# DaviGuanabara/dronechase

Measured on AMD Instinct MI355X. Metric: env-steps/sec (whole job), random-action rollout, higher is better.
Workload: dtype f32

## Files before the change

dronechase_amd/csrc/te_env.hip:

```cpp
#include <hip/hip_runtime.h>
#include <hip/hip_ext.h>

#include <algorithm>
#include <cmath>
#include <cstdio>
#include <cstdlib>
#include <cstring>
#include <map>
#include <mutex>
#include <new>
#include <string>
#include <tuple>
#include <type_traits>
#include <vector>

#include "te_logic.hpp"
#include "te_stacked.hpp"
#include "te_stackview.hpp"
#include "te_engage.hpp"
#include "te_engage_slots.hpp"
#include "te_policy.hpp"
#include "te_policy_bf16.hpp"
#include "te_sphere.hpp"
#include "te_wingman.hpp"
#include "te_policy_grad.hpp"
#include "te_policy_grad_bf16.hpp"
#include "te_policy_opt.hpp"
#include "te_rollout.hpp"
#include "te_monitor.hpp"

namespace te {

#ifndef TE_K1_BLOCK
#define TE_K1_BLOCK 64
#endif
constexpr long long kHelpMaxPairs = 98304;
#ifdef TE_K1_WAVES
#define TE_K1_ATTR __attribute__((amdgpu_waves_per_eu(TE_K1_WAVES, TE_K1_WAVES)))
#else
#define TE_K1_ATTR
#endif
typedef uint32_t te_u4 __attribute__((ext_vector_type(4)));
struct FillJob { float* lidar; uint32_t total_quads; uint32_t n_fill_waves; uint32_t mode; const uint16_t* prev; uint32_t lists, list_rows, npad, n, tile_words; };

struct NavView {
  const SlotLane& P; int Pn;
  TE_DEV float gf(int w, int s) const { return P.lf_slot(TE_X_REF + (w - TE_D_OBS_POS), s); }
};

constexpr int kEagerP = 4;
struct RegNav {
  float ref[3][kEagerP];
  TE_DEV float gf(int w, int s) const {
    float v = 0.0f;
#pragma unroll
    for (int q = 0; q < kEagerP; ++q) v = s == q ? ref[w - TE_D_OBS_POS][q] : v;
    return v;
  }
};
template <int FAMILY, bool NOISE, bool MIXED, bool CES = true, bool HELP = false, bool EAGER = false>
TE_DEV void fly(const Params& p, const float* __restrict__ actions, int slot, int env, bool valid, const float* nzbuf = nullptr, const volatile int* ready = nullptr, uint32_t gate = 1u) {
  const int D = p.D;
  const SlotLane P(p.dstate, p.estate, (uint32_t)D, (uint32_t)p.Npad, (uint32_t)slot, (uint32_t)env,
                   (uint32_t)(TE_DRONE_WORDS + TE_X_WORDS) * (uint32_t)D * (uint32_t)p.Npad, (uint32_t)TE_ENV_WORDS * (uint32_t)p.Npad);
  int armed = EAGER ? 0 : P.li(TE_D_ARMED);
  const bool want = EAGER ? valid : (valid && armed != 0);
  const te_config& c = p.cfg;
  const bool mode7 = (FAMILY == FAM_STAGE01) && slot == 2;
  uint32_t nav_S = 0u; int nav_state = 0; V3 nav_me{0, 0, 0}; RegNav rnav;
#pragma unroll
  for (int k = 0; k < 3; ++k)
#pragma unroll
    for (int q = 0; q < kEagerP; ++q) rnav.ref[k][q] = 0.0f;

  float4 act = make_float4(0, 0, 0, 0);
  float cmd[4] = {0, 0, 0, 0};
// ... 134 lines not shown
#undef TE_DRAW

  const M3 R = x_rotation(b.q);
  if (!c.observe_lag) {
    b.o_pos = b.pos; b.o_vel = mulT(R, b.vel); b.o_rate = b.wb; b.o_eul = euler_of(b.q);
  }
  const V3 ww = mul(R, b.wb);
  P.sf(TE_D_POS, b.pos.x); P.sf(TE_D_POS + 1, b.pos.y); P.sf(TE_D_POS + 2, b.pos.z);
  P.sf(TE_D_QUAT, b.q.x); P.sf(TE_D_QUAT + 1, b.q.y); P.sf(TE_D_QUAT + 2, b.q.z); P.sf(TE_D_QUAT + 3, b.q.w);
  P.sf(TE_D_VEL, b.vel.x); P.sf(TE_D_VEL + 1, b.vel.y); P.sf(TE_D_VEL + 2, b.vel.z);
  P.sf(TE_D_OMEGA, ww.x); P.sf(TE_D_OMEGA + 1, ww.y); P.sf(TE_D_OMEGA + 2, ww.z);
#pragma unroll
  for (int k = 0; k < 4; ++k) P.sf(TE_D_THROTTLE + k, b.thr[k]);
#pragma unroll
  for (int k = 0; k < 3; ++k) { P.sf(TE_D_PID_AV_I + k, b.av_i[k]); P.sf(TE_D_PID_AV_E + k, b.av_e[k]); }
#pragma unroll
  for (int k = 0; k < 2; ++k) { P.sf(TE_D_PID_LV_I + k, b.lv_i[k]); P.sf(TE_D_PID_LV_E + k, b.lv_e[k]); }
  P.sf(TE_D_PID_ZV_I, b.zv_i); P.sf(TE_D_PID_ZV_E, b.zv_e);
  P.sf(TE_D_OBS_POS, b.o_pos.x); P.sf(TE_D_OBS_POS + 1, b.o_pos.y); P.sf(TE_D_OBS_POS + 2, b.o_pos.z);
  P.sf(TE_D_OBS_EULER, b.o_eul.x); P.sf(TE_D_OBS_EULER + 1, b.o_eul.y); P.sf(TE_D_OBS_EULER + 2, b.o_eul.z);
  P.sf(TE_D_OBS_VEL, b.o_vel.x); P.sf(TE_D_OBS_VEL + 1, b.o_vel.y); P.sf(TE_D_OBS_VEL + 2, b.o_vel.z);
  P.sf(TE_D_OBS_RATE, b.o_rate.x); P.sf(TE_D_OBS_RATE + 1, b.o_rate.y); P.sf(TE_D_OBS_RATE + 2, b.o_rate.z);
  if (mode7) {
#pragma unroll
    for (int k = 0; k < 6; ++k) P.sf(TE_D_PENDING + k, 0.0f);
  }
}

#ifdef TE_DEBUG_STAMPS
#define TE_K1_BASE(p) (64 + 16 * (size_t)((p).Npad / kEPB + 1))
#define TE_K1_BEGIN const unsigned long long k1_t0_ = __builtin_amdgcn_s_memrealtime();
#define TE_K1_END(kind)                                                                                               \
  do {                                                                                                                \
    if (p.dbg && threadIdx.x == 0) {                                                                                  \
      asm volatile("s_waitcnt vmcnt(0) lgkmcnt(0)" ::: "memory");                                                    \
      unsigned long long* r_ = p.dbg + TE_K1_BASE(p) + 4 * (size_t)blockIdx.x;                                        \
      r_[0] = k1_t0_; r_[1] = __builtin_amdgcn_s_memrealtime();                                                       \
      r_[2] = (unsigned long long)__builtin_amdgcn_s_getreg((31 << 11) | 4) | ((unsigned long long)__builtin_amdgcn_s_getreg((31 << 11) | 20) << 32); \
      r_[3] = (kind);                                                                                                 \
    }                                                                                                                 \
  } while (0)
#else
#define TE_K1_BEGIN
#define TE_K1_END(kind) do {} while (0)
#endif

template <int FAMILY, bool EAGER>
TE_DEV void noise_help(const Params& p, int slot, int env, bool valid, float* nzbuf, volatile int* ready, uint32_t gate) {
  const te_config& c = p.cfg;
  const int lane = threadIdx.x & 63;
  const SlotLane P(p.dstate, p.estate, (uint32_t)p.D, (uint32_t)p.Npad, (uint32_t)slot, (uint32_t)env,
                   (uint32_t)(TE_DRONE_WORDS + TE_X_WORDS) * (uint32_t)p.D * (uint32_t)p.Npad, (uint32_t)TE_ENV_WORDS * (uint32_t)p.Npad);
  const int armed = P.li(TE_D_ARMED);
  const uint32_t episode = (uint32_t)P.lei(TE_E_EPISODE);
  const uint32_t step_index = (uint32_t)P.lei(TE_E_STEP) + (FAMILY == FAM_STAGE01 ? 1u : 0u);
  if (EAGER) {
    if (!gate) return;
    if (lane == 0) *ready = 0;
    asm volatile("s_waitcnt lgkmcnt(0)\n\ts_barrier" ::: "memory");
  }
  if (__ballot(valid && armed != 0) == 0ull) return;
  const int S = c.substeps;
  for (int s = 0; s < S; s += 2) {
    const U4 bits = motor_noise_bits(c, env, slot, episode, step_index, s);
    float nz[4];
    motor_noise_from(bits.x, bits.y, p.kd.noise_m2ln2, nz);
    *reinterpret_cast<float4*>(nzbuf + ((size_t)s * 64 + lane) * 4) = make_float4(nz[0], nz[1], nz[2], nz[3]);
    if (s + 1 < S) {
      motor_noise_from(bits.z, bits.w, p.kd.noise_m2ln2, nz);
      *reinterpret_cast<float4*>(nzbuf + ((size_t)(s + 1) * 64 + lane) * 4) = make_float4(nz[0], nz[1], nz[2], nz[3]);
    }
    asm volatile("s_waitcnt lgkmcnt(0)" ::: "memory");
    if (lane == 0) *ready = min(s + 2, S);
  }
}

template <int FAMILY, bool NOISE, bool FILL, bool CES = true, bool HELP = false>
__global__ __launch_bounds__(HELP ? 128 : TE_K1_BLOCK) TE_K1_ATTR void substeps_kernel(Params p, const float* __restrict__ actions, FillJob fill) {
  TE_K1_BEGIN
  extern __shared__ float k1_lds[];
  int wave = HELP ? (int)blockIdx.x : __builtin_amdgcn_readfirstlane((int)((blockIdx.x * (unsigned)TE_K1_BLOCK + threadIdx.x) >> 6));
  const int role = HELP ? __builtin_amdgcn_readfirstlane((int)(threadIdx.x >> 6)) : 0;
  volatile int* ready = reinterpret_cast<volatile int*>(k1_lds + (HELP ? (size_t)p.cfg.substeps * 256 : 0));
  const int lane = threadIdx.x & 63;
  const int D = p.D;
  const int nchunks = p.Npad >> 6;
  float4* fill_dst = reinterpret_cast<float4*>(fill.lidar);
  if (FILL) {
    if (HELP && role == 1 && wave < (int)fill.n_fill_waves) return;
    if (wave < (int)fill.n_fill_waves && fill.mode == 3) {
      const uint32_t nch = fill.npad >> 6;
      const uint32_t list = (uint32_t)wave / nch, env = ((uint32_t)wave - list * nch) * 64u + (uint32_t)lane;
      if (env < fill.n) {
        const uint16_t* __restrict__ pv = fill.prev + (size_t)list * fill.list_rows * fill.npad + env;
        float* d0 = fill.lidar + ((size_t)env * fill.lists + list) * fill.tile_words;
        const int cnt = (int)pv[0];
        const bool time_plane = fill.tile_words > 2u * TE_LIDAR_CELLS;
        for (int pl = 0; pl < (time_plane ? 3 : 2); ++pl)
          for (int i = 0; i < cnt; ++i) d0[pl * TE_LIDAR_CELLS + pv[(size_t)(1 + i) * fill.npad]] = 1.0f;
      }
      TE_K1_END(1);
      return;
    }
    if (wave < (int)fill.n_fill_waves) {
      if (fill.mode >= 1) {
        const uint32_t n_blocks = fill.total_quads >> 6;
        const __amdgpu_buffer_rsrc_t rs = __builtin_amdgcn_make_buffer_rsrc(fill.lidar, 0, (int)(n_blocks << 10), 0x00020000);
        const int voff = lane * 16;
        const te_u4 ones = {0x3f800000u, 0x3f800000u, 0x3f800000u, 0x3f800000u};
        for (uint32_t b = (uint32_t)wave; b < n_blocks; b += fill.n_fill_waves)
          __builtin_amdgcn_raw_buffer_store_b128(ones, rs, voff, (int)(b << 10), 2 );
        const uint32_t q = (n_blocks << 6) + (uint32_t)lane;
        if ((uint32_t)wave == n_blocks % fill.n_fill_waves && q < fill.total_quads) TE_FILL_STORE(fill_dst + q);
        TE_K1_END(1);
        return;
      }
      const uint32_t stride = fill.n_fill_waves * 64u;
      for (uint32_t q = (uint32_t)wave * 64u + (uint32_t)lane; q < fill.total_quads; q += stride) TE_FILL_STORE(fill_dst + q);
      TE_K1_END(1);
      return;
    }
    wave -= (int)fill.n_fill_waves;
  }
  const int n_head = min(D, p.cfg.n_pursuers + 1) * nchunks;
  const int n_mixed = (FAMILY == FAM_LEVEL4 && p.dense_min > 1) ? kMixedWaves * nchunks : 0;
  if (wave >= n_head && wave < n_head + n_mixed) {
    wave -= n_head;
    const int m = wave / nchunks, chunk = wave - m * nchunks;
    const int count = __builtin_amdgcn_readfirstlane((int)((const uint32_t* __restrict__)p.mixed_count)[chunk]);
    if (m * 64 >= count) { TE_K1_END(0); return; }
    const int i = m * 64 + lane;
    const bool valid = i < count;
    const uint32_t item = valid ? (uint32_t)p.mixed_items[(size_t)chunk * kMixedCap + i] : 0u;
    if (HELP && role == 1) { noise_help<FAMILY, true>(p, (int)(item >> 8), chunk * 64 + (int)(item & 63u), valid, k1_lds, ready, 1u); return; }
    fly<FAMILY, NOISE, true, CES, HELP, HELP>(p, actions, (int)(item >> 8), chunk * 64 + (int)(item & 63u), valid, k1_lds, ready);
    TE_K1_END(3);
    return;
  }
  if (wave >= n_head) wave -= n_mixed;
  const int slot = wave / nchunks;
  const int chunk = wave - slot * nchunks;
  if (slot >= D) { TE_K1_END(0); return; }
  const uint32_t* __restrict__ sm32 = reinterpret_cast<const uint32_t*>(p.slot_mask);
  const uint32_t chunk_mask = __builtin_amdgcn_readfirstlane(sm32[2 * chunk + (slot >> 5)]);
  const int env = chunk * 64 + lane;
  if (HELP && FAMILY == FAM_LEVEL4) {
    const uint32_t gate = (chunk_mask >> (slot & 31)) & 1u;
// ... 269 lines not shown
}
__global__ void init_planes(Params p) {
  for (size_t i = blockIdx.x * (size_t)blockDim.x + threadIdx.x; i < (size_t)p.D * p.Npad; i += (size_t)gridDim.x * blockDim.x)
    reinterpret_cast<float*>(p.dstate)[(size_t)(TE_D_QUAT + 3) * p.D * p.Npad + i] = 1.0f;
}
__global__ void random_actions_kernel(Params p, float* __restrict__ actions, uint64_t seed, uint64_t step_index) {
  int env = blockIdx.x * blockDim.x + threadIdx.x;
  if (env >= p.N) return;
  uint64_t g = (uint64_t)p.cfg.env_index_base + (uint64_t)env;
  U4 r = philox4x32_10((uint32_t)g, RNG_ACTION | ((uint32_t)(g >> 32) << 24), (uint32_t)step_index, (uint32_t)(step_index >> 32),
                       (uint32_t)seed, (uint32_t)(seed >> 32));
  reinterpret_cast<float4*>(actions)[env] = make_float4(-1.0f + 2.0f * u01(r.x), -1.0f + 2.0f * u01(r.y), -1.0f + 2.0f * u01(r.z), u01(r.w));
}

}

using namespace te;

template <typename... Args> struct Launch { void (*fn)(Args...) = nullptr; const char* name = ""; unsigned block = 0; size_t lds = 0; };
#define TE_KERNEL(...) &__VA_ARGS__, #__VA_ARGS__

struct KernelPlan {
  Launch<Params, const float*, FillJob> substeps[2];
  Launch<Params, const float*, StepOut> engage;
  Launch<StackParams> ring_push;
  Launch<StackParams, StackOut> stack_view;
  size_t observe_lds = 0;
  Launch<Params, int, float*, float*, float*, uint8_t*> wingman_one;
  Launch<Params, int, float*, uint32_t, uint32_t, float*, float*, uint8_t*, uint32_t*> wingman_view;
  Launch<Params, float*, const uint32_t*> wingman_patch;
  uint32_t wingman_fill_waves = 256;
  bool records_cells = false;
  int n_fill_waves = 256, dense_min = kDenseMin;
};
static int family_of(int task) {
  return task == TE_TASK_STAGE01 ? FAM_STAGE01 : (task == TE_TASK_STAGE02 ? FAM_STAGE02 : FAM_LEVEL4);
}
template <typename F>
static void launch_by_family(int family, F&& f) {
  switch (family) {
    case FAM_STAGE01: f(std::integral_constant<int, FAM_STAGE01>{}); break;
    case FAM_STAGE02: f(std::integral_constant<int, FAM_STAGE02>{}); break;
    default: f(std::integral_constant<int, FAM_LEVEL4>{}); break;
  }
}
template <typename F> static void with_bool(bool b, F&& f) { if (b) f(std::true_type{}); else f(std::false_type{}); }
template <int FAMILY, bool NOISE, bool FILL, bool CES, bool HELP>
static Launch<Params, const float*, FillJob> substep_role(const te_config& c) {
  static const std::string name = "substeps_kernel<" + std::to_string(FAMILY) + (NOISE ? ", true" : ", false") + (FILL ? ", true" : ", false") +
                                  (CES ? ", true" : ", false") + (HELP ? ", true>" : ", false>");
  return {&substeps_kernel<FAMILY, NOISE, FILL, CES, HELP>, name.c_str(), HELP ? 128u : (unsigned)TE_K1_BLOCK, HELP ? (size_t)c.substeps * 1024 + 16 : 0};
}

static const char* check_config(const te_config* cfg) {
  if (cfg->struct_size != sizeof(te_config)) return "te_create: te_config.struct_size mismatch (ABI skew)";
  const int D = cfg->n_pursuers + cfg->n_invaders;
  if (cfg->n_envs < 1) return "te_create: n_envs < 1";
  if (cfg->n_pursuers < 1 || cfg->n_invaders < 1 || D > kMaxD64 || cfg->n_pursuers > 31) return "te_create: need 1 <= P <= 31, 1 <= I, P + I <= 64";
  if (cfg->initial_invaders < 0 || cfg->invaders_per_round < 0) return "te_create: initial_invaders / invaders_per_round must not be negative";
  if (cfg->substeps < 0 || cfg->substeps > 255) return "te_create: substeps out of range";
  if (cfg->substeps == 0 && cfg->observe_lag != 0) return "te_create: substeps == 0 (no physics) needs observe_lag == 0";
  if (cfg->task < TE_TASK_STAGE01 || cfg->task > TE_TASK_LEVEL5_FUSION) return "te_create: unknown task";
  if (cfg->ground_contact && family_of(cfg->task) != FAM_LEVEL4) return "te_create: cfg.ground_contact is built for the level4 task family only";
  if (cfg->evaluation && (((uint32_t)cfg->evaluation >> 8) >> cfg->n_pursuers) != 0u) return "te_create: cfg.evaluation's driver mask names a pursuer that does not exist";
  if (cfg->evaluation && !(family_of(cfg->task) == FAM_LEVEL4 && cfg->ally_policy == TE_ALLY_BT && !cfg->stacked_obs))
    return "te_create: cfg.evaluation (Evaluation_Task rules) is the level4 task family with behaviour-tree drivers and the own-sphere observation";
// ... 51 lines not shown
  else if (spw && !c.stacked_obs) k.engage = {TE_KERNEL(engage_slots_multi_kernel<2, true, false>), multi_block, multi_lds};
  else if (spw == 1) k.engage = {TE_KERNEL(engage_slots_multi_kernel<1, false, false>), multi_block, multi_lds};
  else if (spw == 2) k.engage = {TE_KERNEL(engage_slots_multi_kernel<2, false, false>), multi_block, multi_lds};
  else if (spw == 3) k.engage = {TE_KERNEL(engage_slots_multi_kernel<3, false, false>), multi_block, multi_lds};
  else if (regs_s2 && !eng_regs) k.engage = {TE_KERNEL(engage_slots_stage02_kernel<16>), 64u * D, slot_lds};
  else if (slots) k.engage = {TE_KERNEL(engage_slots_kernel<16>), 64u * D, slot_lds};
#ifndef TE_DEBUG_STAMPS
  else if (contact && P <= 2 && D <= 11) k.engage = {TE_KERNEL(engage_kernel<2, 9, true>), 64, 0};
  else if (contact) k.engage = {TE_KERNEL(engage_kernel<6, 12, true>), 64, 0};
#endif
  else if (regs_l4 && P <= 2 && D <= 11) k.engage = {TE_KERNEL(engage_kernel<2, 9, false>), 64, 0};
  else if (regs_l4 && P <= 6 && D <= 18) k.engage = {TE_KERNEL(engage_kernel<6, 12, false>), 64, 0};
  else if (regs_l4) k.engage = {TE_KERNEL(engage_kernel<7, 30, false>), 64, 0};
  else if (regs_s2) k.engage = {TE_KERNEL(engage_stage02_kernel<2, 8>), 64, 0};
  else if (regs_s1) k.engage = {TE_KERNEL(engage_stage01_kernel), 64, 0};
  else if (l4 && lds > 53 * 1024) k.engage = {TE_KERNEL(engage_observe_kernel<0, 512>), 512, lds};
  else if (l4) k.engage = {TE_KERNEL(engage_observe_kernel<0, 256>), 256, lds};
  else if (fam == FAM_STAGE01) k.engage = {TE_KERNEL(engage_observe_kernel<1, 256>), 256, lds};
  else k.engage = {TE_KERNEL(engage_observe_kernel<2, 256>), 256, lds};
  k.observe_lds = lds;
  k.records_cells = !c.stacked_obs && (regs_l4 || regs_s2 || regs_s1);
  const bool help_ok = c.motor_noise && c.substeps >= 2 && c.substeps <= 48 && P <= kEagerP;
  const bool typical_light = l4 && chunks * std::min(D, P + 2) <= 1280;
  bool help = help_ok && ((long long)c.n_envs * D <= kHelpMaxPairs || typical_light);
  if (const char* v = getenv("TE_K1_HELP")) help = atoi(v) != 0 && help_ok;
  launch_by_family(fam, [&](auto F) { with_bool(c.motor_noise != 0, [&](auto N) { with_bool(c.control_every_substep != 0, [&](auto C) { with_bool(help, [&](auto H) {
    constexpr int kF = decltype(F)::value;
    constexpr bool kN = decltype(N)::value, kC = decltype(C)::value, kH = decltype(H)::value;
    if constexpr (kN || !kH) k.substeps[0] = substep_role<kF, kN, false, kC, kH>(c), k.substeps[1] = substep_role<kF, kN, true, kC, kH>(c);
  }); }); }); });
  if (const char* v = getenv("TE_DENSE_MIN")) { const int n = atoi(v); if (n >= 1 && n <= 65) k.dense_min = n; }
  if (c.stacked_obs) k.n_fill_waves = 512;
  if (const char* v = getenv("TE_FILL_WAVES")) { const int n = atoi(v); if (n >= 1 && n <= (1 << 20)) k.n_fill_waves = n; }
  if (c.stacked_obs) {
    const char* stacked = getenv("TE_STACKED");
    const int dm = stacked && !strcmp(stacked, "lds") ? 0 : D <= 18 ? 18 : D <= 37 ? 37 : 0;
    bool split = dm == 18 && chunks * P * kPushSplit <= 4096;
    if (const char* v = getenv("TE_PUSH_SPLIT")) split = dm == 18 && atoi(v) != 0;
    const size_t view_lds = (size_t)view_lds_rows(D) * kEPB * sizeof(uint32_t);
    if (dm == 18 && split) k.ring_push = {TE_KERNEL(ring_push_kernel<18, 4>), 64 * kPushSplit, (size_t)4 * 18 * 256};
    else if (dm == 18) k.ring_push = {TE_KERNEL(ring_push_kernel<18, 1>), 64, 0};
    else if (dm == 37) k.ring_push = {TE_KERNEL(ring_push_kernel<37, 1>), 64, 0};
    if (dm == 18) k.stack_view = {TE_KERNEL(stack_view_kernel<18>), kViewThreads, view_lds};
    else if (dm == 37) k.stack_view = {TE_KERNEL(stack_view_kernel<37>), kViewThreads, view_lds};
    else k.stack_view = {TE_KERNEL(stacked_kernel), kStackThreads, (size_t)stack_lds_rows(D, P) * kEPB * sizeof(uint32_t)};
    k.records_cells = dm != 0;
  }
  if (c.ally_policy == TE_ALLY_EXTERNAL || ((uint32_t)c.evaluation >> 8) != 0u) {
    const size_t n_floats = (size_t)c.n_envs * lidar_words(c);
    k.wingman_one = {TE_KERNEL(observe_ally_kernel), 256, 0};
    if (c.n_envs >= 4096 && (n_floats & 3) == 0 && (n_floats >> 2) < (1ull << 32)) {
      k.wingman_view = {TE_KERNEL(ally_view_kernel), 64, 0};
      k.wingman_patch = {TE_KERNEL(ally_patch_kernel), 256, 0};
    }
  }
  return nullptr;
}

struct te_env {
  Params p;
  int device;
  int family;
  KernelPlan k;
  size_t dbg_words = 0;
  float* zero_actions = nullptr;
  uint32_t* ally_scratch = nullptr;
  struct HostStage {
    char* base = nullptr;
    float *actions = nullptr, *lidar = nullptr, *inertial = nullptr, *last_action = nullptr, *reward = nullptr;
    float *t_lidar = nullptr, *t_inertial = nullptr, *t_last_action = nullptr;
    uint8_t *done = nullptr, *mask = nullptr; int32_t* info = nullptr; uint32_t* blob = nullptr;
    float* t_gather = nullptr;
  } hs;
  std::vector<int32_t> done_idx;
  std::vector<char> done_rows;
  std::vector<hipEvent_t> events;
  int prof_cap = 0, prof_used = 0;
  bool persist_on = false; uint16_t* prev_cells = nullptr; const float* last_stacked = nullptr; int prev_observers = 0, last_n_obs = 0;
  bool prof_markers = false;
};

static thread_local std::string g_err;
static void launch_census(te_env* e, hipStream_t st);
extern "C" __attribute__((visibility("default"))) void te_destroy(te_env* e);
static int fail(const std::string& m) { g_err = m; return 1; }
#define TE_HIP(x)                                                                                      \
  do {                                                                                                 \
    hipError_t e_ = (x);                                                                               \
    if (e_ != hipSuccess) return fail(std::string(#x) + ": " + hipGetErrorString(e_));                  \
  } while (0)

struct DeviceGuard {
  int prev = -1; bool ok;
  explicit DeviceGuard(int dev) { ok = hipGetDevice(&prev) == hipSuccess && (prev == dev || hipSetDevice(dev) == hipSuccess); if (prev == dev) prev = -1; }
  ~DeviceGuard() { if (prev >= 0) (void)hipSetDevice(prev); }
};

static void launch_census(te_env* e, hipStream_t st) {
// ... 156 lines not shown
  TE_HIP(hipGetDeviceCount(&ndev));
  if (ndev < 1) return fail("te_create: no HIP device visible; this library has no CPU fallback");
  if (device_id < 0 || device_id >= ndev) return fail("te_create: bad device_id");
  DeviceGuard guard(device_id);
  if (!guard.ok) return fail("te_create: hipSetDevice failed");
  te_env* e = new (std::nothrow) te_env();
  if (!e) return fail("te_create: out of host memory");
  e->device = device_id;
  e->p.dstate = nullptr; e->p.estate = nullptr; e->p.slot_mask = nullptr; e->p.live_mask = nullptr; e->p.mixed_count = nullptr; e->p.mixed_items = nullptr; e->p.stage_tab = nullptr; e->p.snap = nullptr; e->p.ring = nullptr; e->p.dbg = nullptr;
  auto bail = [&](const std::string& why) { te_destroy(e); return fail(why); };
#define TE_HIP_OR_BAIL(x)                                                                              \
  do {                                                                                                 \
    hipError_t e_ = (x);                                                                               \
    if (e_ != hipSuccess) return bail(std::string("te_create: " #x ": ") + hipGetErrorString(e_));      \
  } while (0)
  if (const char* why = plan_kernels(*cfg, &e->k)) return bail(why);
  e->family = family_of(cfg->task);
  e->p.cfg = *cfg;
  e->p.kd = derive(*cfg);
  e->p.N = cfg->n_envs; e->p.D = D; e->p.Npad = (cfg->n_envs + 63) / 64 * 64;
  e->p.dense_min = e->k.dense_min;
  hipError_t le = set_lds_limits(e->k);
  if (le != hipSuccess && e->k.engage.lds > 64 * 1024) {
    (void)hipGetLastError(); plan_kernels(*cfg, &e->k, 64 * 1024); le = set_lds_limits(e->k);
  }
  if (le != hipSuccess) return bail(std::string("te_create: this many drones per env needs more LDS than a workgroup may have: ") + hipGetErrorString(le));
  const size_t dwords = (size_t)(TE_DRONE_WORDS + TE_X_WORDS) * D * e->p.Npad, ewords = (size_t)TE_ENV_WORDS * e->p.Npad;
  if (hipMalloc(&e->p.dstate, dwords * 4) != hipSuccess || hipMalloc(&e->p.estate, ewords * 4) != hipSuccess)
    return bail("te_create: hipMalloc failed");
  if (hipMalloc(&e->p.slot_mask, (size_t)(e->p.Npad / 64) * 8) != hipSuccess || hipMalloc(&e->p.live_mask, (size_t)(e->p.Npad / 64) * 8) != hipSuccess || hipMalloc(&e->p.mixed_count, (size_t)(e->p.Npad / 64) * 4) != hipSuccess ||
      hipMalloc(&e->p.mixed_items, (size_t)(e->p.Npad / 64) * kMixedCap * sizeof(uint16_t)) != hipSuccess)
    return bail("te_create: hipMalloc failed");
  TE_HIP_OR_BAIL(hipMemsetAsync(e->p.mixed_count, 0, (size_t)(e->p.Npad / 64) * 4, nullptr));
  {
    const Rows r{D, cfg->n_pursuers};
    std::vector<uint32_t> tab((size_t)r.staged());
    for (int row = 0; row < r.staged(); ++row) tab[(size_t)row] = staged_row_offset(e->p, r, row);
    if (hipMalloc(&e->p.stage_tab, tab.size() * 4) != hipSuccess ||
        hipMemcpy(e->p.stage_tab, tab.data(), tab.size() * 4, hipMemcpyHostToDevice) != hipSuccess)
      return bail("te_create: hipMalloc failed");
  }
  if (e->k.wingman_view.fn) {
    if (hipMalloc(&e->ally_scratch, (size_t)2 * D * e->p.Npad * 4) != hipSuccess) return bail("te_create: hipMalloc failed");
  }
  if (cfg->io_location == TE_IO_HOST) {
    const size_t N = (size_t)cfg->n_envs, lw = (size_t)lidar_words(*cfg) * 4;
    const size_t blob = (N * ((size_t)D * TE_DRONE_WORDS + TE_ENV_WORDS)) * 4;
    const size_t sizes[12] = {N * 16, N * lw, N * 60, N * 16, N * 4, N * lw, N * 60, N * 16, N, N, N * 16, blob};
    size_t off[13]; off[0] = 0;
    for (int k = 0; k < 12; ++k) off[k + 1] = off[k] + ((sizes[k] + 255) & ~(size_t)255);
    if (hipMalloc(&e->hs.base, off[12]) != hipSuccess) return bail("te_create: hipMalloc failed (host I/O staging)");
    char* b = e->hs.base;
    e->hs.actions = (float*)(b + off[0]); e->hs.lidar = (float*)(b + off[1]); e->hs.inertial = (float*)(b + off[2]);
    e->hs.last_action = (float*)(b + off[3]); e->hs.reward = (float*)(b + off[4]); e->hs.t_lidar = (float*)(b + off[5]);
    e->hs.t_inertial = (float*)(b + off[6]); e->hs.t_last_action = (float*)(b + off[7]); e->hs.done = (uint8_t*)(b + off[8]);
    e->hs.mask = (uint8_t*)(b + off[9]); e->hs.info = (int32_t*)(b + off[10]); e->hs.blob = (uint32_t*)(b + off[11]);
  }
  e->p.entry_words = TE_RING_ENTRY_WORDS(D);
  if (cfg->stacked_obs && (cfg->agent_scripted || cfg->evaluation)) {
    if (hipMalloc(&e->zero_actions, (size_t)e->p.Npad * 16) != hipSuccess) return bail("te_create: hipMalloc failed");
    TE_HIP_OR_BAIL(hipMemsetAsync(e->zero_actions, 0, (size_t)e->p.Npad * 16, nullptr));
  }
  if (cfg->stacked_obs) {
    const size_t snap_bytes = (size_t)snap_words(D, cfg->n_pursuers) * e->p.Npad * 4;
    const size_t ring_bytes = (size_t)cfg->n_envs * cfg->n_pursuers * TE_RING_DEPTH * e->p.entry_words * 4;
    if (hipMalloc(&e->p.snap, snap_bytes) != hipSuccess || hipMalloc(&e->p.ring, ring_bytes) != hipSuccess)
// ... 13 lines not shown
  const int blocks = (e->p.N + 255) / 256;
  launch_by_family(e->family, [&](auto fam) {
    hipLaunchKernelGGL((reset_kernel<decltype(fam)::value>), dim3(blocks), dim3(256), 0, nullptr, e->p, (const uint8_t*)nullptr);
  });
  launch_census(e, nullptr);
  TE_HIP_OR_BAIL(hipGetLastError());
  TE_HIP_OR_BAIL(hipStreamSynchronize(nullptr));
#undef TE_HIP_OR_BAIL
  *out = e;
  return 0;
}

__attribute__((visibility("default"))) int te_kernel_plan(const te_config* cfg, char* out, size_t out_bytes) {
  if (!cfg || !out) return fail("te_kernel_plan: null argument");
  KernelPlan k;
  const char* why = check_config(cfg);
  if (why || (why = plan_kernels(*cfg, &k))) return fail(why);
  std::string s = std::string("substeps=") + k.substeps[1].name + "\nsubsteps_nofill=" + k.substeps[0].name + "\nengage=" + k.engage.name + "\n" +
                  (k.ring_push.fn ? std::string("ring_push=") + k.ring_push.name + "\n" : "") + (k.stack_view.fn ? std::string("stack_view=") + k.stack_view.name + "\n" : "");
  if (k.wingman_view.fn) s += std::string("wingman_view=") + k.wingman_view.name + "+" + k.wingman_patch.name + "\n";
  else if (k.wingman_one.fn) s += std::string("wingman_view=") + k.wingman_one.name + "\n";
  if (s.size() >= out_bytes) return fail("te_kernel_plan: out_bytes too small (" + std::to_string(s.size() + 1) + " needed)");
  memcpy(out, s.c_str(), s.size() + 1);
  return 0;
}

__attribute__((visibility("default"))) void te_destroy(te_env* e) {
  if (!e) return;
  DeviceGuard guard(e->device);
  for (hipEvent_t ev : e->events) (void)hipEventDestroy(ev);
  (void)hipFree(e->p.dstate);
  (void)hipFree(e->p.estate);
  (void)hipFree(e->ally_scratch);
  (void)hipFree(e->zero_actions);
  (void)hipFree(e->hs.base); (void)hipFree(e->hs.t_gather);
  (void)hipFree(e->p.slot_mask); (void)hipFree(e->p.live_mask); (void)hipFree(e->p.mixed_count); (void)hipFree(e->p.mixed_items);
  (void)hipFree(e->p.stage_tab);
  if (e->p.snap) (void)hipFree(e->p.snap);
  if (e->p.ring) (void)hipFree(e->p.ring);
  if (e->prev_cells) (void)hipFree(e->prev_cells);
  if (e->p.dbg) (void)hipFree(e->p.dbg);
  delete e;
}

__attribute__((visibility("default"))) int te_reset(te_env* e, const uint8_t* env_mask, void* stream) {
  if (!e) return fail("te_reset: null env");
  DeviceGuard guard(e->device);
  if (host_io(e) && env_mask) {
    hipStream_t st = (hipStream_t)stream;
    TE_H2D(e->hs.mask, env_mask, (size_t)e->p.N);
    TE_HIP(hipStreamSynchronize(st));
    env_mask = e->hs.mask;
  }
  const int blocks = (e->p.N + 255) / 256;
  launch_by_family(e->family, [&](auto fam) {
    hipLaunchKernelGGL((reset_kernel<decltype(fam)::value>), dim3(blocks), dim3(256), 0, (hipStream_t)stream, e->p, env_mask);
  });
  launch_census(e, (hipStream_t)stream);
  TE_HIP(hipGetLastError());
  return 0;
}

__attribute__((visibility("default"))) int te_wingman_info(te_env* e, int32_t* wingman_info, void* stream) {
  if (!e || !wingman_info) return fail("te_wingman_info: null argument");
  if (!e->p.cfg.evaluation) return fail("te_wingman_info: per-wingman kills are only counted under cfg.evaluation (Evaluation_Task)");
  DeviceGuard guard(e->device);
// ... 50 lines not shown
  if (e->p.cfg.ally_policy != TE_ALLY_EXTERNAL) return fail("te_observe_ally: this te_env's ally is not driven by the caller (cfg.ally_policy != TE_ALLY_EXTERNAL)");
  return te_observe_wingman(e, 1, ally_lidar, ally_inertial, ally_last_action, ally_active, stream);
}

__attribute__((visibility("default"))) int te_set_ally_actions(te_env* e, const float* ally_actions, void* stream) {
  if (!e) return fail("te_set_ally_actions: null env");
  if (e->p.cfg.ally_policy != TE_ALLY_EXTERNAL) return fail("te_set_ally_actions: this te_env's ally is not driven by the caller (cfg.ally_policy != TE_ALLY_EXTERNAL)");
  if (!ally_actions || ((uintptr_t)ally_actions & 15)) return fail("te_set_ally_actions: ally_actions ([N,4] f32, 16-byte aligned) is required");
  return te_set_wingman_actions(e, 1, ally_actions, stream);
}

static int observe_device(te_env* e, float* obs_lidar, float* obs_inertial, float* obs_last_action, void* stream);
__attribute__((visibility("default"))) int te_observe(te_env* e, float* obs_lidar, float* obs_inertial, float* obs_last_action, void* stream) {
  if (!host_io(e)) return observe_device(e, obs_lidar, obs_inertial, obs_last_action, stream);
  DeviceGuard guard(e->device);
  hipStream_t st = (hipStream_t)stream;
  const size_t N = (size_t)e->p.N;
  if (observe_device(e, obs_lidar ? e->hs.lidar : nullptr, obs_inertial ? e->hs.inertial : nullptr, obs_last_action ? e->hs.last_action : nullptr, stream)) return 1;
  TE_D2H(obs_lidar, e->hs.lidar, N * lidar_words(e->p.cfg) * 4); TE_D2H(obs_inertial, e->hs.inertial, N * 60); TE_D2H(obs_last_action, e->hs.last_action, N * 16);
  TE_HIP(hipStreamSynchronize(st));
  return 0;
}
static int observe_device(te_env* e, float* obs_lidar, float* obs_inertial, float* obs_last_action, void* stream) {
  if (!e) return fail("te_observe: null env");
  if (e->p.D > kMaxD) return fail("te_observe: more than 32 drones per env: the observation comes out of te_observe_stacked / te_step_stacked (or te_step_students)");
  if ((obs_lidar && ((uintptr_t)obs_lidar & 15)) || (obs_last_action && ((uintptr_t)obs_last_action & 15)))
    return fail("te_observe: obs_lidar and obs_last_action must be 16-byte aligned");
  DeviceGuard guard(e->device);
  const int blocks = (e->p.N + kEPB - 1) / kEPB;
  if (obs_lidar && obs_lidar == e->last_stacked) e->last_stacked = nullptr;
  hipLaunchKernelGGL(observe_kernel, dim3(blocks), dim3(256), e->k.observe_lds, (hipStream_t)stream, e->p, ObsOut{obs_lidar, obs_inertial, obs_last_action});
  TE_HIP(hipGetLastError());
  return 0;
}

static int step_impl(te_env* e, const float* actions, float* obs_lidar, size_t lidar_words_per_env, float* obs_inertial,
                     float* obs_last_action, float* reward, uint8_t* done, int32_t* info, float* terminal_lidar,
                     float* terminal_inertial, float* terminal_last_action, const StackOut* stack, void* stream, int n_obs = 1) {
  if (!e) return fail("te_step: null env");
  if (!actions || !reward || !done || !info) return fail("te_step: actions, reward, done and info are required");
  if ((e->p.ring != nullptr) != (stack != nullptr))
    return fail(stack ? "te_step_stacked: this te_env was created without cfg.stacked_obs"
                      : "te_step: this te_env keeps a snapshot ring (cfg.stacked_obs); step it with te_step_stacked");
  if (((uintptr_t)actions & 15) || ((uintptr_t)info & 15) || (obs_lidar && ((uintptr_t)obs_lidar & 15)) ||
      (obs_last_action && ((uintptr_t)obs_last_action & 15)) || (terminal_last_action && ((uintptr_t)terminal_last_action & 15)))
    return fail("te_step: actions, info, obs_lidar and the last_action buffers must be 16-byte aligned");
  DeviceGuard guard(e->device);
  hipStream_t st = (hipStream_t)stream;
  const Params& p = e->p;
  const bool prof = e->prof_used + 4 <= e->prof_cap;
  const bool prof_ext = prof && !e->prof_markers;
  hipEvent_t* pev = prof ? &e->events[e->prof_used] : nullptr;
  hipEvent_t ev_a = nullptr, ev_b = nullptr;
  const KernelPlan& k = e->k;
  if (prof && !prof_ext) TE_HIP(hipEventRecord(pev[0], st));
  const int waves = p.D * (p.Npad >> 6);
  FillJob fill{nullptr, 0u, 0u, 0u, nullptr, 0u, 0u, 0u, 0u, 0u};
  const size_t n_floats = (size_t)p.N * lidar_words_per_env;
  int persist = 0;
  if (stack && e->persist_on && n_obs <= e->prev_observers) persist = (obs_lidar && obs_lidar == e->last_stacked && n_obs == e->last_n_obs) ? (n_obs > 1 ? 3 : 1) : 2;
  if (!stack && e->persist_on && obs_lidar) persist = obs_lidar == e->last_stacked ? 1 : 2;
  if (obs_lidar && persist == 1) {
    const uint32_t lists = stack ? (uint32_t)n_obs * TE_STACK_SPHERES : 1u;
    fill = FillJob{obs_lidar, 0u, lists * (uint32_t)(p.Npad >> 6), 3u, e->prev_cells, lists, (uint32_t)p.D, (uint32_t)p.Npad, (uint32_t)p.N, (uint32_t)(lidar_words_per_env / (size_t)lists)};
  } else if (obs_lidar && persist != 3) {
    const size_t quads = n_floats >> 2;
    if (quads >= 4096 && quads < (1ull << 32)) {
      fill = FillJob{obs_lidar, (uint32_t)quads, (uint32_t)k.n_fill_waves, (quads >> 6) < (1u << 22) ? 1u : 0u, nullptr, 0u, 0u, 0u, 0u, 0u};
      if (n_floats & 3) hipLaunchKernelGGL(fill_ones_kernel, dim3(1), dim3(64), 0, st, obs_lidar + (quads << 2), n_floats & 3);
    } else {
      hipLaunchKernelGGL(fill_ones_kernel, dim3(2048), dim3(256), 0, st, obs_lidar, n_floats);
    }
  }
  if (prof_ext) { ev_a = pev[0]; ev_b = pev[1]; }
  const int b1 = (int)fill.n_fill_waves + waves + (e->family == FAM_LEVEL4 && p.dense_min > 1 ? kMixedWaves * (p.Npad >> 6) : 0);
  launch(k.substeps[fill.lidar ? 1 : 0], b1, st, ev_a, ev_b, p, actions, fill);
  if (prof && !prof_ext) { TE_HIP(hipEventRecord(pev[1], st)); TE_HIP(hipEventRecord(pev[2], st)); }
  if (prof_ext) { ev_a = pev[2]; ev_b = stack ? nullptr : pev[3]; }
  const int b2 = (p.N + kEPB - 1) / kEPB;
  StepOut o{reward, done, info, ObsOut{stack ? nullptr : obs_lidar, obs_inertial, obs_last_action},
            ObsOut{stack ? nullptr : terminal_lidar, terminal_inertial, terminal_last_action}, e->prev_cells, stack ? 0 : persist};
  launch(k.engage, b2, st, ev_a, ev_b, p, actions, o);
  if (stack) {
    ev_a = nullptr; ev_b = nullptr;
    StackParams sp{p.cfg, p.snap, p.ring, p.N, p.Npad, p.D, p.entry_words, 1, 0, n_obs, persist, e->prev_cells};
    if (k.ring_push.fn) launch(k.ring_push, (unsigned)b2 * (unsigned)p.cfg.n_pursuers, st, ev_a, ev_b, sp);
    for (int ob = 0; ob < n_obs; ++ob) {
      sp.push = ob == 0 ? 1 : 0; sp.observer = ob;
      if (prof_ext && ob == n_obs - 1) ev_b = pev[3];
      launch(k.stack_view, b2, st, ev_a, ev_b, sp, *stack);
    }
  }
  e->last_stacked = persist ? obs_lidar : nullptr; e->last_n_obs = n_obs;
  if (prof) { if (!prof_ext) TE_HIP(hipEventRecord(pev[3], st)); e->prof_used += 4; }
  TE_HIP(hipGetLastError());
  return 0;
}

__attribute__((visibility("default"))) int te_step(te_env* e, const float* actions, float* obs_lidar, float* obs_inertial,
                                                   float* obs_last_action, float* reward, uint8_t* done, int32_t* info,
                                                   float* terminal_lidar, float* terminal_inertial, float* terminal_last_action,
// ... 929 lines not shown
```

Before: 920.9 million.

## Balance lidar ones-fill across waves with atomic ticket work-stealing

The lidar fill in the substep kernel now statically assigns a head fraction of blocks round-robin and hands out the remaining pieces through per-counter atomic tickets. Early-finishing waves take more pieces, which targets load imbalance when fill waves and simulation waves compete. Counters are double-buffered by parity and reset for the next step, and the path is skipped under stream capture. It adds atomic traffic and inline-asm waitcnt tricks, and correctness depends on the parity reset ordering across launches.

```diff
diff --git a/dronechase_amd/csrc/te_env.hip b/dronechase_amd/csrc/te_env.hip
--- a/dronechase_amd/csrc/te_env.hip
+++ b/dronechase_amd/csrc/te_env.hip
@@ -41,7 +41,45 @@
 #define TE_K1_ATTR
 #endif
 typedef uint32_t te_u4 __attribute__((ext_vector_type(4)));
-struct FillJob { float* lidar; uint32_t total_quads; uint32_t n_fill_waves; uint32_t mode; const uint16_t* prev; uint32_t lists, list_rows, npad, n, tile_words; };
+struct FillJob { float* lidar; uint32_t total_quads; uint32_t n_fill_waves; uint32_t mode; const uint16_t* prev; uint32_t lists, list_rows, npad, n, tile_words;
+                 uint32_t* tickets; uint32_t counters, piece, per, parity, head; };
+constexpr uint32_t kTicketLine = 32;
+constexpr int kMaxTicketCounters = 64;
+
+TE_DEV uint32_t ticket_request(uint32_t* ctr) {
+  uint32_t tv; uint64_t sv;
+  asm volatile("s_mov_b64 %1, exec\n\ts_mov_b64 exec, 1\n\tglobal_atomic_add %0, %2, %3, off sc0\n\ts_mov_b64 exec, %1"
+               : "=&v"(tv), "=&s"(sv) : "v"(ctr), "v"(1u) : "memory");
+  return tv;
+}
+TE_DEV uint32_t ticket_wait(uint32_t tv, uint32_t ahead) {
+  uint32_t got;
+  asm volatile("s_cmp_lt_u32 %2, 63\n\ts_cbranch_scc1 1f\n\ts_waitcnt vmcnt(63)\n\ts_branch 3f\n"
+               "1:\n\ts_cmp_lt_u32 %2, 31\n\ts_cbranch_scc1 2f\n\ts_waitcnt vmcnt(31)\n\ts_branch 3f\n"
+               "2:\n\ts_waitcnt vmcnt(0)\n"
+               "3:\n\tv_mov_b32 %0, %1"
+               : "=&v"(got) : "v"(tv), "s"(__builtin_amdgcn_readfirstlane(ahead)) : "scc", "memory");
+  return __builtin_amdgcn_readfirstlane(got);
+}
+TE_DEV uint32_t fill_by_tickets(const FillJob& fill, uint32_t wave) {
+  const int lane = threadIdx.x & 63;
+  const uint32_t n_blocks = fill.total_quads >> 6, home = wave % fill.counters;
+  const __amdgpu_buffer_rsrc_t rs = __builtin_amdgcn_make_buffer_rsrc(fill.lidar, 0, (int)(n_blocks << 10), 0x00020000);
+  const int voff = lane * 16;
+  const te_u4 ones = {0x3f800000u, 0x3f800000u, 0x3f800000u, 0x3f800000u};
+  uint32_t* ctr = fill.tickets + ((size_t)fill.parity * fill.counters + home) * kTicketLine;
+  uint32_t pieces = 0, ahead = 0;
+  uint32_t pend = ticket_request(ctr);
+  for (uint32_t b = wave; b < fill.head; b += fill.n_fill_waves, ++ahead) __builtin_amdgcn_raw_buffer_store_b128(ones, rs, voff, (int)(b << 10), 2 );
+  for (uint32_t t = ticket_wait(pend, ahead); t < fill.per; t = ticket_wait(pend, ahead)) {
+    pend = ticket_request(ctr);
+    const uint32_t b0 = fill.head + (home * fill.per + t) * fill.piece, b1 = min(b0 + fill.piece, n_blocks);
+    ahead = 0;
+    for (uint32_t b = b0; b < b1; ++b, ++ahead) __builtin_amdgcn_raw_buffer_store_b128(ones, rs, voff, (int)(b << 10), 2 );
+    pieces += 1;
+  }
+  return pieces;
+}
 
 struct NavView {
   const SlotLane& P; int Pn;
@@ -242,17 +280,17 @@
 #define TE_K1_BEGIN const unsigned long long k1_t0_ = __builtin_amdgcn_s_memrealtime();
 #define TE_K1_END(kind)                                                                                               \
   do {                                                                                                                \
-    if (p.dbg && threadIdx.x == 0) {                                                                                  \
+    if (p.dbg && threadIdx.x == 0) {                                                                                \
       asm volatile("s_waitcnt vmcnt(0) lgkmcnt(0)" ::: "memory");                                                    \
       unsigned long long* r_ = p.dbg + TE_K1_BASE(p) + 4 * (size_t)blockIdx.x;                                        \
       r_[0] = k1_t0_; r_[1] = __builtin_amdgcn_s_memrealtime();                                                       \
       r_[2] = (unsigned long long)__builtin_amdgcn_s_getreg((31 << 11) | 4) | ((unsigned long long)__builtin_amdgcn_s_getreg((31 << 11) | 20) << 32); \
-      r_[3] = (kind);                                                                                                 \
+      r_[3] = (kind);                                                                                              \
     }                                                                                                                 \
   } while (0)
 #else
 #define TE_K1_BEGIN
-#define TE_K1_END(kind) do {} while (0)
+#define TE_K1_END(kind) do { (void)(kind); } while (0)
 #endif
 
 template <int FAMILY, bool EAGER>
@@ -318,11 +356,18 @@
         const __amdgpu_buffer_rsrc_t rs = __builtin_amdgcn_make_buffer_rsrc(fill.lidar, 0, (int)(n_blocks << 10), 0x00020000);
         const int voff = lane * 16;
         const te_u4 ones = {0x3f800000u, 0x3f800000u, 0x3f800000u, 0x3f800000u};
-        for (uint32_t b = (uint32_t)wave; b < n_blocks; b += fill.n_fill_waves)
-          __builtin_amdgcn_raw_buffer_store_b128(ones, rs, voff, (int)(b << 10), 2 );
+        uint32_t pieces = 0;
+        if (fill.mode == 4) {
+          if (wave == 0 && (uint32_t)lane < fill.counters)
+            __hip_atomic_store(fill.tickets + ((size_t)(fill.parity ^ 1u) * fill.counters + (uint32_t)lane) * kTicketLine, 0u, __ATOMIC_RELAXED, __HIP_MEMORY_SCOPE_AGENT);
+          pieces = fill_by_tickets(fill, (uint32_t)wave);
+        } else {
+          for (uint32_t b = (uint32_t)wave; b < n_blocks; b += fill.n_fill_waves)
+            __builtin_amdgcn_raw_buffer_store_b128(ones, rs, voff, (int)(b << 10), 2 );
+        }
         const uint32_t q = (n_blocks << 6) + (uint32_t)lane;
         if ((uint32_t)wave == n_blocks % fill.n_fill_waves && q < fill.total_quads) TE_FILL_STORE(fill_dst + q);
-        TE_K1_END(1);
+        TE_K1_END(1 | (unsigned long long)pieces << 8);
         return;
       }
       const uint32_t stride = fill.n_fill_waves * 64u;
@@ -658,6 +703,7 @@
   uint32_t wingman_fill_waves = 256;
   bool records_cells = false;
   int n_fill_waves = 256, dense_min = kDenseMin;
+  int fill_tickets = 1, fill_counters = 8, fill_piece = 64, fill_head_pct = 50;
 };
 static int family_of(int task) {
   return task == TE_TASK_STAGE01 ? FAM_STAGE01 : (task == TE_TASK_STAGE02 ? FAM_STAGE02 : FAM_LEVEL4);
@@ -775,6 +821,10 @@
   if (const char* v = getenv("TE_DENSE_MIN")) { const int n = atoi(v); if (n >= 1 && n <= 65) k.dense_min = n; }
   if (c.stacked_obs) k.n_fill_waves = 512;
   if (const char* v = getenv("TE_FILL_WAVES")) { const int n = atoi(v); if (n >= 1 && n <= (1 << 20)) k.n_fill_waves = n; }
+  if (const char* v = getenv("TE_FILL_TICKETS")) k.fill_tickets = atoi(v) != 0;
+  if (const char* v = getenv("TE_FILL_COUNTERS")) { const int n = atoi(v); if (n >= 1 && n <= kMaxTicketCounters) k.fill_counters = n; }
+  if (const char* v = getenv("TE_FILL_PIECE")) { const int n = atoi(v); if (n >= 1 && n <= 4096) k.fill_piece = n; }
+  if (const char* v = getenv("TE_FILL_HEAD")) { const int n = atoi(v); if (n >= 0 && n <= 100) k.fill_head_pct = n; }
   if (c.stacked_obs) {
     const char* stacked = getenv("TE_STACKED");
     const int dm = stacked && !strcmp(stacked, "lds") ? 0 : D <= 18 ? 18 : D <= 37 ? 37 : 0;
@@ -807,6 +857,8 @@
   KernelPlan k;
   size_t dbg_words = 0;
   float* zero_actions = nullptr;
+  uint32_t* fill_pool = nullptr;
+  uint32_t fill_parity = 0;
   uint32_t* ally_scratch = nullptr;
   struct HostStage {
     char* base = nullptr;
@@ -1029,6 +1081,11 @@
       hipMalloc(&e->p.mixed_items, (size_t)(e->p.Npad / 64) * kMixedCap * sizeof(uint16_t)) != hipSuccess)
     return bail("te_create: hipMalloc failed");
   TE_HIP_OR_BAIL(hipMemsetAsync(e->p.mixed_count, 0, (size_t)(e->p.Npad / 64) * 4, nullptr));
+  if (e->k.fill_tickets) {
+    const size_t pool_bytes = (size_t)2 * e->k.fill_counters * kTicketLine * 4;
+    if (hipMalloc(&e->fill_pool, pool_bytes) != hipSuccess) return bail("te_create: hipMalloc failed");
+    TE_HIP_OR_BAIL(hipMemsetAsync(e->fill_pool, 0, pool_bytes, nullptr));
+  }
   {
     const Rows r{D, cfg->n_pursuers};
     std::vector<uint32_t> tab((size_t)r.staged());
@@ -1108,6 +1165,7 @@
   (void)hipFree(e->p.dstate);
   (void)hipFree(e->p.estate);
   (void)hipFree(e->ally_scratch);
+  (void)hipFree(e->fill_pool);
   (void)hipFree(e->zero_actions);
   (void)hipFree(e->hs.base); (void)hipFree(e->hs.t_gather);
   (void)hipFree(e->p.slot_mask); (void)hipFree(e->p.live_mask); (void)hipFree(e->p.mixed_count); (void)hipFree(e->p.mixed_items);
@@ -1224,6 +1282,11 @@
   hipLaunchKernelGGL(observe_kernel, dim3(blocks), dim3(256), e->k.observe_lds, (hipStream_t)stream, e->p, ObsOut{obs_lidar, obs_inertial, obs_last_action});
   TE_HIP(hipGetLastError());
   return 0;
+}
+
+static bool stream_is_capturing(hipStream_t st) {
+  hipStreamCaptureStatus status = hipStreamCaptureStatusNone;
+  return st != nullptr && (hipStreamIsCapturing(st, &status) != hipSuccess || status != hipStreamCaptureStatusNone);
 }
 
 static int step_impl(te_env* e, const float* actions, float* obs_lidar, size_t lidar_words_per_env, float* obs_inertial,
@@ -1259,6 +1322,15 @@
     const size_t quads = n_floats >> 2;
     if (quads >= 4096 && quads < (1ull << 32)) {
       fill = FillJob{obs_lidar, (uint32_t)quads, (uint32_t)k.n_fill_waves, (quads >> 6) < (1u << 22) ? 1u : 0u, nullptr, 0u, 0u, 0u, 0u, 0u};
+      if (e->fill_pool && fill.mode == 1 && !stream_is_capturing(st)) {
+        const uint32_t n_blocks = (uint32_t)(quads >> 6);
+        fill.mode = 4; fill.tickets = e->fill_pool; fill.piece = (uint32_t)k.fill_piece; fill.parity = e->fill_parity;
+        fill.counters = (uint32_t)std::min(k.fill_counters, k.n_fill_waves);
+        fill.head = (uint32_t)((uint64_t)n_blocks * (uint32_t)k.fill_head_pct / 100u);
+        const uint32_t pieces = (n_blocks - fill.head + fill.piece - 1) / fill.piece;
+        fill.per = (pieces + fill.counters - 1) / fill.counters;
+        e->fill_parity ^= 1u;
+      }
       if (n_floats & 3) hipLaunchKernelGGL(fill_ones_kernel, dim3(1), dim3(64), 0, st, obs_lidar + (quads << 2), n_floats & 3);
     } else {
       hipLaunchKernelGGL(fill_ones_kernel, dim3(2048), dim3(256), 0, st, obs_lidar, n_floats);
```

Result: slower. 902.9 million (-2.0%).
